# cheshmi/parsy_bench

Measured on AMD Instinct MI355X. Metric: Cholesky factorizations/sec (+ SpTRSV solves/sec), SuiteSparse SPD set, higher is better.
Workload: dtype f64; 1 GPU; flan-class stand-in (BASELINE.json configs[2] when flan: Flan_1565): grid (116, 116, 116) 27-point stencil, geometric nested dissection; n=1560896, nnz_A_lower=21491316, nsuper=81191, nnz_L=2044454227, xsize=2421483055, etree_levels=17, launches_per_factorization=356, parallelism=1 GPU

## Files before the change

parsy_bench_amd/csrc/schedule.cpp:

```cpp
#include "schedule.hpp"

#include <array>
#include <cstdio>
#include <map>
#include <algorithm>
#include <queue>
#include <climits>
#include <cmath>
#include <cstdlib>
#include <cstdint>
#include <functional>
#include <stdexcept>
#include <string>

namespace parsy {

static inline int ceil_div(int a, int b) { return (a + b - 1) / b; }

static int env_int(const char* name, int dflt) {
    const char* v = std::getenv(name);
    if (!v || !*v) return dflt;
    return std::atoi(v);
}

static int find_subtrees(const std::vector<int>& parent, const std::vector<uint8_t>& eligible,
                         const std::vector<double>& cost, double cap, std::vector<int32_t>& subtree,
                         const std::vector<std::pair<int32_t, int32_t>>* slots = nullptr, int64_t slot_cap = 0) {
    const int ns = (int)parent.size();
    subtree.assign(ns, -1);
    std::vector<uint8_t> whole(eligible);
    std::vector<double> sub(cost);
    std::vector<int64_t> cols(slots ? ns : 0);
    for (int s = 0; s < ns && slots; ++s) cols[s] = (*slots)[s].first;
    for (int s = 0; s < ns; ++s) {
        const int p = parent[s];
        if (p < 0) continue;
        if (p <= s) return 0;
        if (!whole[s]) whole[p] = 0;
        sub[p] += sub[s];
        if (slots) cols[p] += cols[s];
    }
    int count = 0;
    for (int s = ns - 1; s >= 0; --s) {
        const int p = parent[s];
        if (p >= 0 && subtree[p] >= 0) subtree[s] = subtree[p];
        else if (whole[s] && sub[s] <= cap && (!slots || cols[s] + (*slots)[s].second <= slot_cap)) subtree[s] = count++;
    }
    return count;
}

namespace {

struct BuildKnobs {
    bool big_mink_set;
    int big_mink;
    bool piece_width_set;
    int piece_width;
    int push_group;
    bool split_chunks_set;
    int split_chunks;
    int split_target;
    int split_max;
    bool subtrees_set;
    int subtrees_per_cu;
    int chol_subtrees_per_cu;
    int super_r, super_c;
    int64_t super_min_tasks;
    double super_max_fill;
    int super_hi;
    int dense_mode;
    double dense_min_share;
    double dense_all_share;
    int dense_fill_min;
    bool dense_strips;
    bool big_recut;
};

BuildKnobs read_build_knobs() {
    auto percent = [](const char* name, double dflt) { return env_int(name, (int)(dflt * 100 + 0.5)); };
    BuildKnobs K{};
    K.big_mink_set = std::getenv("PARSY_BIG_MINK") != nullptr;
    K.big_mink = std::max(1, env_int("PARSY_BIG_MINK", kBigMinK));
    K.piece_width_set = std::getenv("PARSY_PIECE_WIDTH") != nullptr;
    K.piece_width = env_int("PARSY_PIECE_WIDTH", kPieceWidth);
    K.push_group = std::max(1, env_int("PARSY_PUSH_GROUP", kPushGroup));
    K.split_chunks_set = std::getenv("PARSY_SPLIT_CHUNKS") != nullptr;
    K.split_chunks = env_int("PARSY_SPLIT_CHUNKS", kSplitChunks);
    K.split_target = std::max(1, env_int("PARSY_SPLIT_TARGET", kSplitTarget));
    K.split_max = std::max(1, env_int("PARSY_SPLIT_MAX", kSplitMaxParts));
    K.subtrees_set = std::getenv("PARSY_SUBTREES") != nullptr;
    K.subtrees_per_cu = env_int("PARSY_SUBTREES", kSubtreesPerCu);
    K.chol_subtrees_per_cu = std::max(1, env_int("PARSY_CHOL_SUBTREES", kCholSubtreesPerCu));
    if (const char* e = std::getenv("PARSY_BIG_SUPER")) {
        int a = 0, b = 0;
        const int got = std::sscanf(e, "%dx%d", &a, &b);
        if (got >= 1 && a >= 1 && a <= 64) {
            K.super_r = a;
            K.super_c = (got == 2 && b >= 1 && b <= 64) ? b : a;
        }
    }
    K.super_min_tasks = env_int("PARSY_BIG_SUPER_MIN", kBigSuperMinTasks);
    K.super_max_fill = percent("PARSY_BIG_SUPER_FILL", kBigSuperMaxFill) / 100.0;
    K.super_hi = std::max(1, std::min(8, env_int("PARSY_BIG_SUPER_HI", 2)));
    K.dense_mode = env_int("PARSY_BIG_DENSE", 1);
    K.dense_min_share = percent("PARSY_DENSE_MIN_SHARE", kDenseMinShare) / 100.0;
    K.dense_all_share = percent("PARSY_DENSE_ALL_SHARE", kDenseAllShare) / 100.0;
    K.dense_fill_min = percent("PARSY_DENSE_FILL", kDenseMinFill) * kBigTile * kBigTile / 100;
    K.dense_strips = env_int("PARSY_DENSE_STRIPS", 1) != 0;
    K.big_recut = env_int("PARSY_BIG_RECUT", 1) != 0;
    return K;
}

struct BigKeyed { int64_t launch_tile, window; WaveEntry e; int16_t sr, sc; };

struct BuildState {
    BuildKnobs knobs;
    int compute_units = 0;
    std::vector<int> tree;
    std::vector<int64_t> uptr, urel;
    std::vector<int> usn, ulb, uub;
    std::vector<int8_t> launch_super;
    std::vector<int64_t> level_tiles;
    std::vector<int64_t> big_tile0;
    std::vector<int32_t> upd_domain;
    std::vector<BigKeyed> bigk;
};

struct RowRun { int32_t win, first, len; };

inline int rel_at(const Schedule& S, const SnDesc& T, const UpdDesc& U, int k) {
    return U.rel < 0 ? k : S.relpos[(size_t)U.rel + k] - T.rbias;
}

void row_runs(const Schedule& S, const SnDesc& T, const UpdDesc& U, int window, std::vector<RowRun>& out) {
    out.clear();
    for (int k = 0; k < U.m;) {
        const int win = rel_at(S, T, U, k) / window;
        int k1 = k + 1;
        while (k1 < U.m && rel_at(S, T, U, k1) / window == win) ++k1;
        out.push_back(RowRun{win, k, k1 - k});
        k = k1;
    }
}

inline bool is_big(const Schedule& S, const UpdDesc& U, int target_piece) {
    const int real = S.csn_real[target_piece];
    return U.rel < 0 || U.K >= S.big_min_k || S.piece0[real + 1] - S.piece0[real] > 1;
}

inline int64_t big_launch_of(int lev_s, int lev_t) { return (int64_t)lev_s * 2 + (lev_s == lev_t - 1 ? 0 : 1); }

double block_pairs(int ia, int mi, int ja, int nj) {
    double pairs = 0;
    for (int jj = ja; jj < ja + nj; ++jj) pairs += std::max(0, ia + mi - std::max(ia, jj));
    return pairs;
}

void describe_supernodes(const PatternRef& P, const size_t* lC, const int* A2p, Schedule& S) {
    const int n = P.n, ns = P.nsuper;
    S.n = n;
    S.nsuper = ns;
    S.solve_only = (A2p == nullptr);
    S.nnzA = A2p ? A2p[n] : 0;
    S.rows.assign(P.s, P.s + P.i_ptr[n]);
    S.ssize = (int64_t)P.i_ptr[n];
    S.xsize = (int64_t)lC[n];
    S.sn.resize(ns);
    for (int t = 0; t < ns; ++t) {
        SnDesc& d = S.sn[t];
        d.c0 = P.super[t];
        d.w = P.super[t + 1] - P.super[t];
        d.r = (int)(P.i_ptr[P.super[t + 1]] - P.i_ptr[P.super[t]]);
        d.ld = d.r;
        d.rbias = 0;
        d.px = (int64_t)lC[d.c0];
        d.pi = (int64_t)P.i_ptr[d.c0];
        d.a0 = A2p ? A2p[d.c0] : 0;
        d.a1 = A2p ? A2p[P.super[t + 1]] : 0;
        d.upd0 = 0;
        d.nupd = 0;
        d.dslot = -1;
        d.tflag0 = -1;
        if (d.w <= 0 || d.r < d.w) throw std::runtime_error("schedule: malformed supernode");
        if ((int64_t)d.w * d.r > 0x7fffffffLL)
            throw std::runtime_error("schedule: a single panel exceeds 2^31 entries");
        for (int col = d.c0; col < d.c0 + d.w; ++col)
            if (lC[col + 1] - lC[col] != (size_t)d.r || P.i_ptr[col] != P.i_ptr[d.c0])
                throw std::runtime_error("schedule: lC / Li_ptr are not a column-major panel layout");
        S.max_width = std::max(S.max_width, d.w);
        S.max_rows = std::max(S.max_rows, d.r);
        S.nnzL += (int64_t)d.w * d.r - (int64_t)d.w * (d.w - 1) / 2;
        for (int k = 0; k < d.w; ++k) S.flops_stored += (double)(d.r - k) * (double)(d.r - k);
        for (int k = 0; k < d.w; ++k)
            if (S.rows[d.pi + k] != d.c0 + k)
                throw std::runtime_error("schedule: supernode rows do not start with its own columns");
        if (d.w > kTile) {
            d.dslot = (int32_t)S.n_dslots;
            S.n_dslots += ceil_div(d.w, kTile);
        }
    }
}

void list_updates(const PatternRef& P, const size_t* lC, const int* A2p, const int* A2i, Schedule& S, BuildState& B) {
    const int n = P.n, ns = P.nsuper;
    B.uptr.assign(ns + 1, 0);
    if (!S.solve_only) build_update_lists(P, B.uptr, B.usn, B.ulb, B.uub);
    B.urel.assign(B.usn.size(), 0);
// ... 300 lines not shown
                    rg[part * 8 + 2 * q + 1] = e;
                }
            }
            tsplit[tp / 2] = (int64_t)S.split_desc.size();
            S.split_desc.push_back(sd);
        }
    }
}

void build_wave_streams(Schedule& S, BuildState& B) {
    const int nc = (int)S.csn.size();
    S.sn_wp0.assign(nc, -1);
    S.sn_tw0.assign(nc, -1);
    B.level_tiles.assign((size_t)std::max(S.cnlevels, 1), 0);
    if (S.solve_only) return;
    for (int t = 0; t < nc; ++t)
        if (!is_small(S.csn[t])) {
            const int nbc = ceil_div(S.csn[t].w, kTile), nbr = ceil_div(S.csn[t].r, kTile);
            B.level_tiles[(size_t)S.level_of[t]] += (int64_t)nbc * nbr - (int64_t)nbc * (nbc - 1) / 2;
        }
    std::vector<RowRun> runs;
    std::vector<int64_t> cursor;
    for (int t = 0; t < nc; ++t) {
        SnDesc& T = S.csn[t];
        if (is_small(T)) {
            S.n_small++;
            continue;
        }
        S.n_big++;
        const int nbc = ceil_div(T.w, kTile), nbr = ceil_div(T.r, kTile);
        if (S.n_tflags + (int64_t)nbc * nbr > 0x7fffffffLL) throw std::runtime_error("schedule: too many tiles");
        T.tflag0 = (int32_t)S.n_tflags;
        S.n_tflags += (int64_t)nbc * nbr;
        for (int jb = 1; jb < nbc; ++jb) {
            const double K = (double)jb * kTile, wb = std::min(kTile, T.w - jb * kTile);
            S.inner_flops += K * wb * (wb + 1) + 2.0 * K * (double)(T.r - jb * kTile - wb) * wb;
        }
        piece_wave_streams(S, t, runs, cursor);
        piece_tile_weights(S, B, t);
    }
}

template <class Fn>
void tile_cut_blocks(const Schedule& S, const SnDesc& T, const UpdDesc& U, int sr, int sc, std::vector<RowRun>& runs,
                     std::vector<RowRun>& cruns, Fn&& fn) {
    row_runs(S, T, U, kBigTile * sr, runs);
    if (sc == sr) cruns = runs;
    else row_runs(S, T, U, kBigTile * sc, cruns);
    for (const RowRun& gc : cruns) {
        if (gc.first >= U.n1) break;
        const int njt = std::min(gc.len, U.n1 - gc.first);
        for (const RowRun& gr : runs) {
            if ((int64_t)(gr.win + 1) * sr * kBigTile - 1 < (int64_t)gc.win * sc * kBigTile) continue;
            for (int cb = 0; cb < njt; cb += kBigTile)
                for (int rb = 0; rb < gr.len; rb += kBigTile) {
                    const int mi = std::min(kBigTile, gr.len - rb), nj = std::min(kBigTile, njt - cb);
                    const int ia = gr.first + rb, ja = gc.first + cb;
                    if (ia + mi - 1 < ja) continue;
                    fn(gr.win, gc.win, ia, mi, ja, nj);
                }
        }
    }
}

template <class Fn>
void recut_blocks(const UpdDesc& U, bool strips, Fn&& fn) {
    strips = strips && U.K >= kDenseChunk;
    for (int ja = 0; ja < U.n1; ja += kBigTile)
        for (int ia = ja; ia < U.m; ia += kBigTile) {
            const int mi = std::min(kBigTile, U.m - ia), nj = std::min(kBigTile, U.n1 - ja);
            const bool row_strip = strips && mi <= kStripMax && nj == kBigTile && ia >= ja + kBigTile;
            const bool col_strip = strips && !row_strip && nj <= kStripMax && mi == kBigTile && ja >= kBigTile;
            fn(ia / kBigTile - row_strip, ja / kBigTile - col_strip, ia, mi, ja, nj, row_strip || col_strip);
        }
}

int64_t issued_ns(const BuildKnobs& K, int mi, int nj, int k, bool rides) {
    if (rides) return (int64_t)ceil_div(k, kDenseChunk) * kIssueStripNs;
    const bool dense = K.dense_mode != 0 && k >= kDenseChunk && (K.dense_mode == 4 || mi * nj >= K.dense_fill_min);
    if (dense) return (int64_t)ceil_div(k, kDenseChunk) * kIssueDenseNs;
    return (int64_t)ceil_div(k, 16) * (kIssueRaggedNs + (int64_t)kIssueFragmentNs * ceil_div(mi, 16) * ceil_div(nj, 16));
}

void find_conflict_domains(Schedule& S, BuildState& B) {
    const BuildKnobs& K = B.knobs;
    const int nc = (int)S.csn.size();
    B.upd_domain.assign(S.upd.size(), 0);
    if (S.solve_only || !K.big_recut) return;
    std::vector<std::pair<int64_t, int64_t>> big;
    std::vector<int64_t> owner;
    std::vector<int32_t> root;
    std::vector<std::pair<int32_t, int32_t>> members;
    std::vector<RowRun> runs, cruns;
    auto find = [&](int32_t x) {
        while (root[(size_t)x] != x) x = root[(size_t)x] = root[(size_t)root[(size_t)x]];
        return x;
    };
    for (int t = 0; t < nc; ++t) {
        const SnDesc& T = S.csn[t];
        if (is_small(T)) continue;
        big.clear();
        for (int64_t u = T.upd0; u < T.upd0 + T.nupd; ++u)
            if (is_big(S, S.upd[u], t)) big.push_back({big_launch_of(S.level_of[S.upd_src[u]], S.level_of[t]), u});
        std::stable_sort(big.begin(), big.end(), [](const auto& a, const auto& b) { return a.first < b.first; });
        owner.assign((size_t)T.w, -1);
        for (size_t i = 0; i < big.size();) {
            size_t j = i;
            while (j < big.size() && big[j].first == big[i].first) ++j;
            const int64_t launch = big[i].first;
            const int32_t nm = (int32_t)(j - i);
            root.resize((size_t)nm);
            for (int32_t q = 0; q < nm; ++q) {
                root[(size_t)q] = q;
                const UpdDesc& U = S.upd[big[i + q].second];
                for (int k = 0; k < U.n1; ++k) {
                    const int c = rel_at(S, T, U, k);
                    if (c < 0 || c >= T.w) throw std::runtime_error("schedule: a column row of an update lies outside its target");
                    int64_t& o = owner[(size_t)c];
                    if (o < 0 || (o >> 32) != launch) {
                        o = (launch << 32) | q;
                        continue;
                    }
                    const int32_t a = find(q), b = find((int32_t)(o & 0xffffffff));
                    if (a < b) root[(size_t)b] = a;
                    else root[(size_t)a] = b;
                }
            }
            const int sr = K.super_r ? K.super_r : B.launch_super[(size_t)launch];
            const int sc = K.super_r ? K.super_c : B.launch_super[(size_t)launch];
            members.clear();
            for (int32_t q = 0; q < nm; ++q) members.push_back({find(q), q});
            std::sort(members.begin(), members.end());
            for (size_t d0 = 0, d1; d0 < members.size(); d0 = d1) {
                const int32_t q = members[d0].first;
                for (d1 = d0; d1 < members.size() && members[d1].first == q; ++d1) {}
                const UpdDesc& U0 = S.upd[big[i + q].second];
                bool same = true;
                for (size_t d = d0 + 1; d < d1 && same; ++d) {
                    const UpdDesc& U = S.upd[big[i + members[d].second].second];
                    same = U.m == U0.m && U.n1 == U0.n1;
                    for (int k = 0; k < U.m && same; ++k) same = rel_at(S, T, U, k) == rel_at(S, T, U0, k);
                }
                if (!same) continue;
                int64_t tile_ns = 0, recut_ns = 0;
                for (size_t d = d0; d < d1; ++d) {
                    const UpdDesc& U = S.upd[big[i + members[d].second].second];
                    tile_cut_blocks(S, T, U, sr, sc, runs, cruns, [&](int, int, int, int mi, int, int nj) {
                        tile_ns += issued_ns(K, mi, nj, U.K, false);
                    });
                    recut_blocks(U, K.dense_strips && K.dense_mode != 0, [&](int, int, int, int mi, int, int nj, bool rides) {
                        recut_ns += issued_ns(K, mi, nj, U.K, rides);
                    });
                }
                if (recut_ns >= tile_ns) continue;
                const int64_t first = big[i + q].second - T.upd0;
                if (first >= 0x7fffffff) throw std::runtime_error("schedule: too many updates of one piece");
                for (size_t d = d0; d < d1; ++d) B.upd_domain[(size_t)big[i + members[d].second].second] = (int32_t)first + 1;
            }
            i = j;
        }
    }
}

void collect_big_entries(Schedule& S, BuildState& B) {
    const int nc = (int)S.csn.size();
    const int env_sr = B.knobs.super_r, env_sc = B.knobs.super_c;
    B.big_tile0.assign((size_t)nc + 1, 0);
    std::vector<RowRun> runs, cruns;
    for (int t = 0; t < nc; ++t) {
        const SnDesc& T = S.csn[t];
        B.big_tile0[t + 1] = B.big_tile0[t];
        if (S.solve_only || is_small(T)) continue;
        const int lev_t = S.level_of[t];
        const int nbr128 = ceil_div(T.r, kBigTile), nbc128 = ceil_div(T.w, kBigTile);
        B.big_tile0[t + 1] = B.big_tile0[t] + (int64_t)nbr128 * nbc128;
        for (int64_t u = T.upd0; u < T.upd0 + T.nupd; ++u) {
            const UpdDesc& U = S.upd[u];
            const double f = (double)U.K * U.n1 * (U.n1 + 1) + 2.0 * U.K * (double)(U.m - U.n1) * U.n1;
            if (!is_big(S, U, t)) {
                S.tile_update_flops += f;
                continue;
            }
            S.big_flops += f;
            const int lev_s = S.level_of[S.upd_src[u]];
            if (lev_s >= lev_t) throw std::runtime_error("schedule: an update source is not below its target");
            const int64_t launch = big_launch_of(lev_s, lev_t);
            const int sr = env_sr ? env_sr : B.launch_super[(size_t)launch], sc = env_sr ? env_sc : B.launch_super[(size_t)launch];
            auto entry = [&](int ia, int mi, int ja, int nj) {
                return WaveEntry{U.src, (int32_t)std::max<int64_t>(U.rel, 0), U.ld, U.K, ia, ja, mi | (nj << 8) | ((U.rel < 0) << 16)};
            };
            const int64_t domain = B.upd_domain[(size_t)u];
            if (domain) {
                if (U.m / kBigTile >= 0xffff) throw std::runtime_error("schedule: too many windows of one update");
                recut_blocks(U, B.knobs.dense_strips && B.knobs.dense_mode != 0, [&](int wr, int wc, int ia, int mi, int ja, int nj, bool) {
                    B.bigk.push_back(BigKeyed{(launch << 40) | B.big_tile0[t], (domain << 32) | ((int64_t)wc << 16) | wr,
                                              entry(ia, mi, ja, nj), 1, 1});
                });
                continue;
            }
            tile_cut_blocks(S, T, U, sr, sc, runs, cruns, [&](int wr, int wc, int ia, int mi, int ja, int nj) {
                const int64_t tile = B.big_tile0[t] + (int64_t)wc * sc * nbr128 + (int64_t)wr * sr;
                B.bigk.push_back(BigKeyed{(launch << 40) | tile, 0, entry(ia, mi, ja, nj), (int16_t)sr, (int16_t)sc});
            });
        }
    }
}

std::vector<uint8_t> dense_share_per_launch(const BuildState& B) {
    const BuildKnobs& K = B.knobs;
    std::vector<double> lprod(B.launch_super.size(), 0.0), ldense(B.launch_super.size(), 0.0);
    for (const BigKeyed& b : B.bigk) {
        const WaveEntry& E = b.e;
        const size_t l = (size_t)(b.launch_tile >> 40);
        const double products = (double)ceil_div(E.K, 4) * ceil_div(entry_rows(E), 16) * ceil_div(entry_cols(E), 16);
        lprod[l] += products;
        if (entry_rows(E) == kBigTile && entry_cols(E) == kBigTile && E.K >= kDenseChunk) ldense[l] += products;
    }
    std::vector<uint8_t> launch_dense(B.launch_super.size(), 0);
    for (size_t l = 0; l < launch_dense.size(); ++l) {
        if (K.dense_mode == 4) {
            launch_dense[l] = lprod[l] > 0 ? 2 : 0;
            continue;
        }
        if (K.dense_mode == 0 || ldense[l] <= 0) continue;
        if (K.dense_mode >= 2 || ldense[l] >= K.dense_min_share * lprod[l]) launch_dense[l] = 1;
        if (launch_dense[l] && lprod[l] - ldense[l] <= K.dense_all_share * lprod[l] && K.dense_mode != 3) launch_dense[l] = 2;
    }
    return launch_dense;
}

void build_big_tasks(Schedule& S, BuildState& B) {
    std::vector<BigKeyed>& bigk = B.bigk;
    if (bigk.empty()) return;
    const int nc = (int)S.csn.size();
    std::stable_sort(bigk.begin(), bigk.end(),
                     [](const BigKeyed& a, const BigKeyed& b) {
                         return a.launch_tile != b.launch_tile ? a.launch_tile < b.launch_tile : a.window < b.window;
                     });
    const std::vector<uint8_t> launch_dense = dense_share_per_launch(B);
    const int fill_min = B.knobs.dense_fill_min;
    auto is_dense = [fill_min](const WaveEntry& E, int mode) {
        if (mode == 2) return E.K >= kDenseChunk;
        return mode == 1 && E.K >= kDenseChunk && entry_rows(E) * entry_cols(E) >= fill_min;
    };
    S.big_entries.resize(bigk.size());
    std::map<std::pair<int64_t, int64_t>, size_t> strip_of;
    std::vector<uint8_t> absorbed;
    int t = 0;
    for (size_t i = 0; i < bigk.size();) {
        size_t j = i;
        while (j < bigk.size() && bigk[j].launch_tile == bigk[i].launch_tile && bigk[j].window == bigk[i].window) ++j;
        const int64_t launch = bigk[i].launch_tile >> 40, tile = bigk[i].launch_tile & ((1LL << 40) - 1);
        size_t at = i;
        int64_t weight = 0, dweight = 0, dchunks = 0;
        const int lmode = launch_dense[(size_t)launch];
        const bool strips_ride = bigk[i].window != 0 && lmode == 2 && B.knobs.dense_strips;
        auto dense_here = [&](const WaveEntry& E) {
            if (!is_dense(E, lmode)) return false;
            const int mi = entry_rows(E), nj = entry_cols(E);
            return !(strips_ride && ((mi <= kStripMax && nj == kBigTile) || (nj <= kStripMax && mi == kBigTile)));
        };
        if (lmode)
            for (size_t q = i; q < j; ++q) {
                const WaveEntry& E = bigk[q].e;
                if (!dense_here(E)) continue;
                S.big_entries[at++] = E;
                dchunks += ceil_div(E.K, kDenseChunk);
                dweight += ceil_div(E.K, 16) + 2;
                S.dense_flops += 2.0 * E.K * block_pairs(E.ia, entry_rows(E), E.ja, entry_cols(E));
            }
        const size_t mid = at;
        int32_t nstrips = 0;
        absorbed.assign(j - i, 0);
        if (lmode && B.knobs.dense_strips && mid > i) {
            strip_of.clear();
            for (size_t d = i; d < mid; ++d) {
                const WaveEntry& E = S.big_entries[d];
                if ((E.mn & 0xffff) == (kBigTile | (kBigTile << 8))) strip_of[{E.src, ((int64_t)E.ia << 32) | (uint32_t)E.ja}] = d;
            }
            for (size_t q = i; q < j && !strip_of.empty(); ++q) {
                const WaveEntry& R = bigk[q].e;
                if (dense_here(R)) continue;
                const int mi = entry_rows(R), nj = entry_cols(R);
                const bool row_strip = mi <= kStripMax && nj == kBigTile, col_strip = nj <= kStripMax && mi == kBigTile;
                if (!row_strip && !col_strip) continue;
                const auto it = strip_of.find({R.src, ((int64_t)(R.ia - (row_strip ? kBigTile : 0)) << 32) |
                                                      (uint32_t)(R.ja - (col_strip ? kBigTile : 0))});
                if (it == strip_of.end()) continue;
                WaveEntry& E = S.big_entries[it->second];
                if (E.K != R.K || big_ident(E) != big_ident(R) || E.rel != R.rel || E.ld != R.ld) continue;
                if ((row_strip ? big_strip_rows(E) : big_strip_cols(E)) != 0) continue;
                if (big_strip_rows(E) == 0 && big_strip_cols(E) == 0) ++nstrips;
                E.mn |= row_strip ? mi << 17 : nj << 22;
                absorbed[q - i] = 1;
                S.dense_flops += 2.0 * R.K * block_pairs(R.ia, mi, R.ja, nj);
                dweight += ceil_div(R.K, 64);
            }
        }
        for (size_t q = i; q < j; ++q)
            if (!dense_here(bigk[q].e) && !absorbed[q - i]) {
                S.big_entries[at++] = bigk[q].e;
                weight += ceil_div(bigk[q].e.K, 16) + 4;
            }
        const size_t jend = at;
        S.n_dense_entries += (int64_t)(mid - i);
        S.n_strip_entries += nstrips;
        while (t + 1 < nc && B.big_tile0[t + 1] <= tile) ++t;
        if (tile < B.big_tile0[t]) {
            t = 0;
            while (B.big_tile0[t + 1] <= tile) ++t;
        }
        const int nbr128 = ceil_div(S.csn[t].r, kBigTile);
        const int64_t local = tile - B.big_tile0[t];
        const int64_t window = bigk[i].window;
        const int32_t row0 = window ? (int32_t)(window & 0xffff) * kBigTile : (int32_t)(local % nbr128) * kBigTile;
        const int32_t col0 = window ? (int32_t)((window >> 16) & 0xffff) * kBigTile : (int32_t)(local / nbr128) * kBigTile;
        S.big_all.push_back(Schedule::BigTask{t, row0, col0,
                                              (int32_t)std::min<int64_t>(weight, INT32_MAX), (int64_t)i, (int64_t)jend,
                                              (int32_t)(launch >> 1), (int32_t)((launch & 1) == 0), bigk[i].sr, bigk[i].sc,
                                              (int64_t)mid, (int32_t)std::min<int64_t>(dweight, INT32_MAX),
                                              (int32_t)std::min<int64_t>(dchunks, INT32_MAX), nstrips, (int32_t)(window >> 32)});
        i = j;
    }
}

}

void build_schedule(const PatternRef& P, const size_t* lC, const int* A2p, const int* A2i,
                    const uint8_t* active, Schedule& S, int compute_units) {
    S = Schedule();
    BuildState B;
    B.knobs = read_build_knobs();
    B.compute_units = compute_units;
    if (compute_units > 0) S.walker_batch = std::max(4, std::min(kWalkerBatch, compute_units / 2));
    describe_supernodes(P, lC, A2p, S);
    list_updates(P, lC, A2p, A2i, S, B);
    choose_sizes(S, B.knobs);
    cut_pieces(P, S, B);
    describe_updates(S, B);
// ... 1350 lines not shown
            if (l.rows_only != 0 && !(l.rows_only == 1 && k == kLaunchChain)) fail(who + "rows_only is set");
            if (l.ticket != 0 && !(k == kLaunchChain || chain_form)) fail(who + "has a ticket counter but takes no tickets");
            if (l.ticket < 0 || (l.ticket > 0 && l.ticket >= ntickets)) fail(who + "ticket counter " + std::to_string(l.ticket) + " does not exist");
            if ((l.lds_bytes != 0 || l.stage != 0) && k != kLaunchSmall) fail(who + "lds_bytes / stage are set");
            if (l.lds_bytes < 0 || l.stage < 0) fail(who + "negative lds_bytes / stage");
            if (l.width != 0 && k != kLaunchSolveSmall) fail(who + "width is set");
            if (l.width_class < 0 || l.width_class > 2 || (l.width_class != 0 && k != kLaunchBackBlock))
                fail(who + "width_class = " + std::to_string(l.width_class));
            if ((l.task_first != 0 || l.task_count != 0) && !chain_form) fail(who + "has a task range but is no chain-form launch");
        }
    };
    check_list(S.chol, "chol", [](int k) { return is_chol_launch(k); }, S.n_chain_launches);
    check_list(S.solve, "solve", [](int k) { return k == kLaunchSolveSmall || k == kLaunchSolvePanel || k == kLaunchSolveFixup; },
               S.n_solve_chain_launches);
    check_list(S.bsolve, "bsolve", [](int k) { return k == kLaunchBackBelow || k == kLaunchBackBlock; }, S.n_solve_chain_launches);
}

int64_t check_schedule(const Schedule& S, std::string& what) {
    int64_t bad = 0;
    auto fail = [&](const std::string& msg) {
        if (bad++ == 0) what = msg;
    };
    check_launch_records(S, fail);
    check_solve_launches(S, fail);
    check_solve_one(S, fail);
    check_sub_tiers(S, fail);
    if (S.solve_only) return bad;
    const int nc = (int)S.csn.size();
    for (int t = 0; t < S.nsuper; ++t) {
        int cols = 0;
        for (int p = S.piece0[t]; p < S.piece0[t + 1]; ++p) {
            const SnDesc& C = S.csn[p];
            if (C.c0 != S.sn[t].c0 + cols || C.rbias != cols || C.r != S.sn[t].r - cols || C.ld != S.sn[t].r)
                fail("piece " + std::to_string(p) + " is not a window of its supernode's panel");
            if (p > S.piece0[t] && S.level_of[p] != S.level_of[p - 1] + 1) fail("pieces of a supernode are not on consecutive levels");
            cols += C.w;
        }
        if (cols != S.sn[t].w) fail("pieces of supernode " + std::to_string(t) + " do not add up to its width");
    }
    std::vector<double> covered(S.upd.size(), 0.0);
    auto entry_flops = [](const WaveEntry& E, bool same_window) {
        const double K = E.K, mi = E.mn & 255, nj = (E.mn >> 8) & 255;
        return same_window ? K * nj * (nj + 1) + 2.0 * K * (mi - nj) * nj : 2.0 * K * mi * nj;
    };
    auto block_flops = [](const WaveEntry& E) {
        const int mi = E.mn & 255, nj = (E.mn >> 8) & 255;
        auto pairs_of = [](int ia, int m, int ja, int n) {
            double pairs = 0;
            for (int j = ja; j < ja + n; ++j) pairs += std::max(0, ia + m - std::max(ia, j));
            return pairs;
        };
        return 2.0 * E.K * (pairs_of(E.ia, mi, E.ja, nj) + pairs_of(E.ia + mi, big_strip_rows(E), E.ja, nj) +
                            pairs_of(E.ia, mi, E.ja + nj, big_strip_cols(E)));
    };
    for (int t = 0; t < nc; ++t) {
        const SnDesc& T = S.csn[t];
        for (int64_t u = T.upd0; u < T.upd0 + T.nupd; ++u)
            if (S.level_of[S.upd_src[u]] >= S.level_of[t]) fail("update " + std::to_string(u) + " comes from a level that is not below its target");
        if (is_small(T) || T.nupd == 0) continue;
        auto find_upd = [&](const WaveEntry& E) -> int64_t {
            for (int64_t u = T.upd0; u < T.upd0 + T.nupd; ++u)
                if (S.upd[u].src == E.src && S.upd[u].K == E.K) return u;
            return -1;
        };
        if (S.sn_wp0[t] >= 0) {
            const int nbc = ceil_div(T.w, kTile), nbr = ceil_div(T.r, kTile);
            const int64_t* wp = &S.wave_ptr[S.sn_wp0[t]];
            for (size_t key = 0; key < (size_t)nbc * nbr * 8; ++key)
                for (int64_t e = wp[key]; e < wp[key + 1]; ++e) {
                    const WaveEntry& E = S.wave_entries[(size_t)e];
                    const int64_t u = find_upd(E);
                    const int mi = E.mn & 255, nj = (E.mn >> 8) & 255;
                    if (u < 0 || mi < 1 || mi > kSub || nj < 1 || nj > kSub || E.ia + mi > S.upd[u].m || E.ja + nj > S.upd[u].n1) {
                        fail("wave entry " + std::to_string(e) + " of piece " + std::to_string(t) + " has a bad window");
                        continue;
                    }
                    covered[(size_t)u] += entry_flops(E, E.ia == E.ja);
                }
        }
    }
    std::vector<int32_t> col_domain;
    std::map<int32_t, int64_t> domain_upd;
    std::vector<std::array<int32_t, 3>> domain_wins;
    const Schedule::BigTask* group = nullptr;
    auto close_group = [&]() {
        std::sort(domain_wins.begin(), domain_wins.end());
        if (std::adjacent_find(domain_wins.begin(), domain_wins.end()) != domain_wins.end())
            fail("two BIG tasks of piece " + std::to_string(group->sn) + " own the same window of a conflict domain");
        domain_wins.clear();
        domain_upd.clear();
    };
    for (const Schedule::BigTask& b : S.big_all) {
        const SnDesc& T = S.csn[b.sn];
        if (b.src_level >= S.level_of[b.sn] || (b.next != 0) != (b.src_level == S.level_of[b.sn] - 1))
            fail("BIG task of piece " + std::to_string(b.sn) + " is filed under the wrong source level");
        if (!group || group->sn != b.sn || group->src_level != b.src_level || group->next != b.next) {
            if (group) close_group();
            group = &b;
            col_domain.assign((size_t)T.w, -1);
        }
        const int win_r = kBigTile * b.sr, win_c = kBigTile * b.sc;
        if (b.domain < 0 || b.sr < 1 || b.sc < 1 || b.row0 % win_r || b.col0 % win_c || b.row0 + win_r <= b.col0 ||
            (b.domain ? b.sr != 1 || b.sc != 1 : b.row0 >= T.r || b.col0 >= T.w))
            fail("BIG task of piece " + std::to_string(b.sn) + " has a bad tile origin");
        if (b.domain) domain_wins.push_back({b.domain, b.row0, b.col0});
        for (int64_t e = b.e0; e < b.e1; ++e) {
            const WaveEntry& E = S.big_entries[(size_t)e];
            int64_t u = -1;
            for (int64_t q = T.upd0; q < T.upd0 + T.nupd; ++q)
                if (S.upd[q].src == E.src && S.upd[q].K == E.K) u = q;
            const int mi = E.mn & 255, nj = (E.mn >> 8) & 255;
            const bool ident = big_ident(E);
            const int ms = big_strip_rows(E), ns = big_strip_cols(E);
            if ((ms || ns) && (e >= b.em || mi != kBigTile || nj != kBigTile || ms > kStripMax || ns > kStripMax))
                fail("BIG entry " + std::to_string(e) + " carries a strip but is not a full dense block");
            if (u < 0 || mi < 1 || mi > kBigTile || nj < 1 || nj > kBigTile || E.ia + mi + ms > S.upd[u].m || E.ja + nj + ns > S.upd[u].n1 ||
                ident != (S.upd[u].rel < 0) || S.level_of[S.upd_src[u]] != b.src_level) {
                fail("BIG entry " + std::to_string(e) + " of piece " + std::to_string(b.sn) + " has a bad window or source");
                continue;
            }
            auto rel_at = [&](int k) { return ident ? k : S.relpos[(size_t)S.upd[u].rel + k] - T.rbias; };
            for (int k = E.ja; k < E.ja + nj + ns; ++k) {
                int32_t& d = col_domain[(size_t)rel_at(k)];
                if (d >= 0 && d != b.domain)
                    fail("column " + std::to_string(rel_at(k)) + " of piece " + std::to_string(b.sn) + " belongs to two conflict domains of a launch");
                d = b.domain;
            }
            if (!b.domain) {
                if (rel_at(E.ia) / win_r != b.row0 / win_r || rel_at(E.ia + mi + ms - 1) / win_r != b.row0 / win_r ||
                    rel_at(E.ja) / win_c != b.col0 / win_c || rel_at(E.ja + nj + ns - 1) / win_c != b.col0 / win_c)
                    fail("BIG entry " + std::to_string(e) + " names rows outside its task's tile");
            } else {
                const UpdDesc& U = S.upd[u];
                auto inside = [](int first, int count, int win0, int len) {
                    const int end = first + count, wend = win0 + kBigTile;
                    return first >= win0 && (end <= wend || (end <= len && len - wend <= kStripMax));
                };
                if (!inside(E.ia, mi + ms, b.row0, U.m) || !inside(E.ja, nj + ns, b.col0, U.n1))
                    fail("BIG entry " + std::to_string(e) + " names rows outside its task's window");
                const UpdDesc& U0 = S.upd[(size_t)domain_upd.emplace(b.domain, u).first->second];
                bool same = U.m == U0.m && U.n1 == U0.n1 && (U.rel < 0) == (U0.rel < 0);
                if (&U != &U0 && !ident) {
                    for (int k = E.ia; k < E.ia + mi + ms && same; ++k) same = S.relpos[(size_t)U.rel + k] == S.relpos[(size_t)U0.rel + k];
                    for (int k = E.ja; k < E.ja + nj + ns && same; ++k) same = S.relpos[(size_t)U.rel + k] == S.relpos[(size_t)U0.rel + k];
                }
                if (!same) fail("BIG entry " + std::to_string(e) + ": the members of its conflict domain do not have the same rows");
            }
            covered[(size_t)u] += block_flops(E);
        }
    }
    if (group) close_group();
    {
        std::vector<int64_t> starts;
        std::vector<int64_t> dense_pos(S.big_all.size(), -1), ragged_pos(S.big_all.size(), -1);
        int64_t li = 0;
        for (const Launch& l : S.chol) {
            ++li;
            if (l.kind != kLaunchBig && l.kind != kLaunchDense) continue;
            const bool dense = l.kind == kLaunchDense;
            const bool side = l.side != 0;
            auto find_task = [&](int64_t e) -> const Schedule::BigTask* {
                auto it = std::upper_bound(S.big_all.begin(), S.big_all.end(), e,
                                           [](int64_t v, const Schedule::BigTask& b) { return v < b.e0; });
                if (it == S.big_all.begin()) return nullptr;
                --it;
                return e < it->e1 ? &*it : nullptr;
            };
            auto right_launch = [&](const Schedule::BigTask& b) {
                return side != (b.next != 0) && (side ? l.wait_level : l.level - 1) == b.src_level;
            };
            for (int q = l.first; q < l.first + l.count; ++q) {
                const TileDesc& td = S.big_tasks[(size_t)q];
                if (td.wp >= td.sp) {
                    if (td.wp != td.sp) fail("BIG launch task " + std::to_string(q) + " has a negative entry range");
                    continue;
                }
                const Schedule::BigTask* it = find_task(td.wp);
                const bool ok = it && (dense ? (it->e0 == td.wp && it->em == td.sp && (td.part & ~kDenseStripTask) == it->dchunks &&
                                                ((td.part & kDenseStripTask) != 0) == (it->strips > 0))
                                             : (it->em == td.wp && it->e1 == td.sp));
                if (!ok || it->sn != td.sn || it->row0 != td.row0 || it->col0 != td.col0) {
                    fail("BIG launch task " + std::to_string(q) + " is not a task of the plan");
                    continue;
                }
                if (!right_launch(*it)) fail("BIG launch task " + std::to_string(q) + " runs in the launch of another source level");
                (dense ? dense_pos : ragged_pos)[(size_t)(it - S.big_all.data())] = li;
                starts.push_back(td.wp);
            }
        }
        std::sort(starts.begin(), starts.end());
        if (std::adjacent_find(starts.begin(), starts.end()) != starts.end()) fail("a BIG task is launched twice");
        int64_t want = 0;
        for (size_t k = 0; k < S.big_all.size(); ++k) {
            const Schedule::BigTask& b = S.big_all[k];
            if (b.em < b.e0 || b.em > b.e1) fail("BIG task " + std::to_string(k) + " has a bad dense / ragged split");
            int64_t dch = 0;
            int32_t nst = 0;
            for (int64_t e = b.e0; e < b.em; ++e) {
                const WaveEntry& E = S.big_entries[(size_t)e];
                nst += big_strip_rows(E) || big_strip_cols(E);
                if (E.K < kDenseChunk) fail("BIG entry " + std::to_string(e) + " is filed as dense but is narrower than a chunk");
                dch += ceil_div(E.K, kDenseChunk);
            }
            if (dch != b.dchunks) fail("BIG task " + std::to_string(k) + " has a wrong dense chunk count");
            if (nst != b.strips) fail("BIG task " + std::to_string(k) + " has a wrong count of entries with strips");
            if (!S.active_piece[b.sn]) continue;
            want += (b.em > b.e0) + (b.e1 > b.em);
            if (b.em > b.e0 && b.e1 > b.em && !(dense_pos[k] > 0 && ragged_pos[k] > dense_pos[k]))
                fail("BIG task " + std::to_string(k) + ": the ragged part is not launched after the dense part");
        }
        if ((int64_t)starts.size() != want)
            fail("BIG launches hold " + std::to_string(starts.size()) + " task parts, the active targets have " + std::to_string(want));
    }
    for (int t = 0; t < nc; ++t) {
// ... 62 lines not shown
```

parsy_bench_amd/csrc/schedule.hpp:

```cpp
#pragma once
#include <cstddef>
#include <cstdint>
#include <string>
#include <vector>

#include "inspector.hpp"

namespace parsy {

constexpr int kTile = 64;
constexpr int kSub = 32;
constexpr int kSmallMaxEntries = 6144;
constexpr int kSmallMaxWidth = 64;
constexpr int kBelowRows = 512;
constexpr int kBelowMaxGroups = 512;
constexpr int kBackGroup = 2;
constexpr int kTinyWidth = 16;
constexpr int kTinyWidth2 = 32;
constexpr int kPanelRows = 128;
constexpr int kSolveRows = 256;
constexpr int kSolveRowsMrhs = 128;

struct SnDesc {
    int64_t px;
    int64_t pi;
    int64_t upd0;
    int32_t c0, w, r;
    int32_t nupd;
    int32_t a0, a1;
    int32_t dslot;
    int32_t tflag0;
    int32_t ld;
    int32_t rbias;
};

struct UpdDesc {
    int64_t src;
    int64_t rel;
    int32_t ld;
    int32_t K;
    int32_t m;
    int32_t n1;
};

struct WaveEntry {
    int64_t src;
    int32_t rel;
    int32_t ld, K;
    int32_t ia, ja;
    int32_t mn;
};
constexpr int kStripMax = 16;
constexpr int kIssueDenseNs = 2090, kIssueStripNs = 260, kIssueRaggedNs = 1000, kIssueFragmentNs = 60;
inline int entry_rows(const WaveEntry& E) { return E.mn & 255; }
inline int entry_cols(const WaveEntry& E) { return (E.mn >> 8) & 255; }
inline bool big_ident(const WaveEntry& E) { return (E.mn >> 16) & 1; }
inline int big_strip_rows(const WaveEntry& E) { return (E.mn >> 17) & 31; }
inline int big_strip_cols(const WaveEntry& E) { return (E.mn >> 22) & 31; }
constexpr int kDenseStripTask = 1 << 30;

struct TileDesc {
    int32_t sn;
    int32_t row0, col0;
    int32_t part;
    int64_t wp;
    int64_t sp;
};

struct PanelDesc {
    int32_t sn;
    int32_t jb;
    int32_t row0;
    int32_t pad;
};

struct SubMember {
    int64_t px;
    int32_t c0, w, r;
    int32_t slot0;
    int32_t so;
    int32_t ld;
};
struct SubTree {
    int32_t m0, m1;
    int32_t ncols;
    int32_t nout;
    int32_t out0;
    int32_t pad[3];
};
struct SubTier {
    int32_t tree0, ntrees;
    int32_t max_slots;
    int32_t top_level;
};
constexpr int kSubMaxSlots = 320;
constexpr int kSubTierMaxWidth = 64;
constexpr int kSubTierMinTrees = 512;
constexpr int kSubTierMaxSlots = 448;
constexpr int kSubTierMaxDensity = 700;

enum LaunchKind : int32_t {
    kLaunchSmall = 0, kLaunchTiles = 1, kLaunchChain = 2, kLaunchBig = 3,
    kLaunchBackBelow = 4,
    kLaunchSolveSmall = 5, kLaunchSolvePanel = 6, kLaunchSolveFixup = 7, kLaunchBackBlock = 8,
    kLaunchDense = 9,
};
inline bool is_chol_launch(int kind) { return (kind >= 0 && kind <= kLaunchBig) || kind == kLaunchDense; }

enum LaunchForm : int32_t {
    kFormEach = 0,
    kFormChain = 1,
    kFormSubtrees = 2,
};

struct Launch {
    int32_t kind;
    int32_t first = 0, count = 0;
    int32_t level = 0;
    int32_t side = 0;
    int32_t wait_level = -1;
    int32_t form = kFormEach;
    int32_t rows_only = 0;
    int32_t ticket = 0;
    int32_t lds_bytes = 0;
    int32_t stage = 0;
    int32_t width = 0;
    int32_t width_class = 0;
    int32_t task_first = 0, task_count = 0;
};
constexpr int kLaunchFields = 15;
static_assert(sizeof(Launch) == kLaunchFields * sizeof(int32_t), "Launch: fields and kLaunchFields disagree");

constexpr int kSplitChunks = 192;
constexpr int kSplitTarget = 128;
constexpr int kSplitMaxParts = 4;
constexpr int kSplitFewTiles = 128;
// ... 151 lines not shown
```

Measured before the change: 3.036 factorizations/s.

## Recut non-identical BIG update conflict domains into swept row intervals

Adds an interval-based recut mode for conflict domains whose member updates have different row patterns. Row boundaries come from a sweep that caps each update at one block per interval. The cut is used only when its estimated issue cost beats the tiled cut and it does not lengthen the longest task beyond the launch's share across issue slots. The aim is to pack ragged updates into fuller blocks and cut fragment overhead, at the cost of more schedule-build work, a new domain encoding, and checker logic for interval overlap.

```diff
diff --git a/parsy_bench_amd/csrc/schedule.cpp b/parsy_bench_amd/csrc/schedule.cpp
--- a/parsy_bench_amd/csrc/schedule.cpp
+++ b/parsy_bench_amd/csrc/schedule.cpp
@@ -5,6 +5,7 @@
 #include <map>
 #include <algorithm>
 #include <queue>
+#include <set>
 #include <climits>
 #include <cmath>
 #include <cstdlib>
@@ -73,7 +74,8 @@
     double dense_all_share;
     int dense_fill_min;
     bool dense_strips;
-    bool big_recut;
+    bool big_recut_set;
+    int big_recut;
 };
 
 BuildKnobs read_build_knobs() {
@@ -107,7 +109,8 @@
     K.dense_all_share = percent("PARSY_DENSE_ALL_SHARE", kDenseAllShare) / 100.0;
     K.dense_fill_min = percent("PARSY_DENSE_FILL", kDenseMinFill) * kBigTile * kBigTile / 100;
     K.dense_strips = env_int("PARSY_DENSE_STRIPS", 1) != 0;
-    K.big_recut = env_int("PARSY_BIG_RECUT", 1) != 0;
+    K.big_recut_set = std::getenv("PARSY_BIG_RECUT") != nullptr;
+    K.big_recut = std::max(0, std::min(3, env_int("PARSY_BIG_RECUT", 2)));
     return K;
 }
 
@@ -123,6 +126,8 @@
     std::vector<int64_t> level_tiles;
     std::vector<int64_t> big_tile0;
     std::vector<int32_t> upd_domain;
+    std::vector<int64_t> upd_bounds;
+    std::vector<int32_t> bounds;
     std::vector<BigKeyed> bigk;
 };
 
@@ -589,16 +594,95 @@
     return (int64_t)ceil_div(k, 16) * (kIssueRaggedNs + (int64_t)kIssueFragmentNs * ceil_div(mi, 16) * ceil_div(nj, 16));
 }
 
+void interval_bounds(const Schedule& S, const SnDesc& T, const std::vector<const UpdDesc*>& members,
+                     std::vector<std::pair<int32_t, int32_t>>& rows, std::vector<int32_t>& count, std::vector<int32_t>& bounds) {
+    rows.clear();
+    for (size_t q = 0; q < members.size(); ++q)
+        for (int k = 0; k < members[q]->m; ++k) rows.push_back({rel_at(S, T, *members[q], k), (int32_t)q});
+    std::sort(rows.begin(), rows.end());
+    count.assign(members.size(), 0);
+    bounds.assign(1, 0);
+    for (size_t a = 0, b; a < rows.size(); a = b) {
+        const int32_t pos = rows[a].first;
+        for (b = a; b < rows.size() && rows[b].first == pos; ++b) {}
+        int32_t start = 0;
+        if (pos >= T.w && bounds.back() < T.w) start = T.w;
+        for (size_t c = a; c < b && !start; ++c)
+            if (count[(size_t)rows[c].second] == kBigTile) start = pos;
+        if (start) {
+            bounds.push_back(start);
+            std::fill(count.begin(), count.end(), 0);
+        }
+        for (size_t c = a; c < b; ++c) ++count[(size_t)rows[c].second];
+    }
+}
+
+template <class Fn>
+void interval_blocks(const Schedule& S, const SnDesc& T, const UpdDesc& U, const int32_t* bounds, int nb, std::vector<RowRun>& runs,
+                     Fn&& fn) {
+    runs.clear();
+    int w = 0;
+    for (int k = 0; k < U.m;) {
+        const int pos = rel_at(S, T, U, k);
+        while (w + 1 < nb && bounds[w + 1] <= pos) ++w;
+        int k1 = k + 1;
+        while (k1 < U.m && (w + 1 >= nb || rel_at(S, T, U, k1) < bounds[w + 1])) ++k1;
+        if (k1 - k > kBigTile) throw std::runtime_error("schedule: an interval holds more than a block of one update's rows");
+        runs.push_back(RowRun{w, k, k1 - k});
+        k = k1;
+    }
+    for (const RowRun& gc : runs) {
+        if (gc.first >= U.n1) break;
+        const int nj = std::min(gc.len, U.n1 - gc.first);
+        for (const RowRun& gr : runs) {
+            if (gr.win < gc.win || gr.first + gr.len - 1 < gc.first) continue;
+            fn(gr.win, gc.win, gr.first, gr.len, gc.first, nj);
+        }
+    }
+}
+
 void find_conflict_domains(Schedule& S, BuildState& B) {
     const BuildKnobs& K = B.knobs;
     const int nc = (int)S.csn.size();
     B.upd_domain.assign(S.upd.size(), 0);
-    if (S.solve_only || !K.big_recut) return;
+    B.upd_bounds.assign(S.upd.size(), -1);
+    B.bounds.clear();
+    const int recut = K.big_recut_set || (S.update_flops >= kPieceAutoFlops && !K.super_r) ? K.big_recut : 1;
+    if (S.solve_only || !recut) return;
+    std::vector<RowRun> runs, cruns;
+    auto super_of = [&](int64_t launch) {
+        return std::pair<int, int>{K.super_r ? K.super_r : B.launch_super[(size_t)launch], K.super_r ? K.super_c : B.launch_super[(size_t)launch]};
+    };
+    std::vector<int64_t> launch_tile_ns(B.launch_super.size(), 0);
+    if (recut == 2)
+        for (int t = 0; t < nc; ++t) {
+            const SnDesc& T = S.csn[t];
+            if (is_small(T)) continue;
+            for (int64_t u = T.upd0; u < T.upd0 + T.nupd; ++u) {
+                const UpdDesc& U = S.upd[u];
+                if (!is_big(S, U, t)) continue;
+                const int64_t launch = big_launch_of(S.level_of[S.upd_src[u]], S.level_of[t]);
+                const auto [sr, sc] = super_of(launch);
+                int64_t ns = 0;
+                tile_cut_blocks(S, T, U, sr, sc, runs, cruns, [&](int, int, int, int mi, int, int nj) { ns += issued_ns(K, mi, nj, U.K, false); });
+                launch_tile_ns[(size_t)launch] += ns;
+            }
+        }
+    std::vector<const UpdDesc*> member_upd;
+    std::vector<std::pair<int32_t, int32_t>> sweep_rows;
+    std::vector<int32_t> sweep_count, ivals;
+    std::map<std::pair<int, int>, int64_t> tile_task, ival_task;
+    std::set<std::array<int, 4>> full_blocks;
+    const bool strips = K.dense_mode != 0;
+    auto longest = [](const std::map<std::pair<int, int>, int64_t>& m) {
+        int64_t v = 0;
+        for (const auto& kv : m) v = std::max(v, kv.second);
+        return v;
+    };
     std::vector<std::pair<int64_t, int64_t>> big;
     std::vector<int64_t> owner;
     std::vector<int32_t> root;
     std::vector<std::pair<int32_t, int32_t>> members;
-    std::vector<RowRun> runs, cruns;
     auto find = [&](int32_t x) {
         while (root[(size_t)x] != x) x = root[(size_t)x] = root[(size_t)root[(size_t)x]];
         return x;
@@ -633,8 +717,7 @@
                     else root[(size_t)a] = b;
                 }
             }
-            const int sr = K.super_r ? K.super_r : B.launch_super[(size_t)launch];
-            const int sc = K.super_r ? K.super_c : B.launch_super[(size_t)launch];
+            const auto [sr, sc] = super_of(launch);
             members.clear();
             for (int32_t q = 0; q < nm; ++q) members.push_back({find(q), q});
             std::sort(members.begin(), members.end());
@@ -648,7 +731,48 @@
                     same = U.m == U0.m && U.n1 == U0.n1;
                     for (int k = 0; k < U.m && same; ++k) same = rel_at(S, T, U, k) == rel_at(S, T, U0, k);
                 }
-                if (!same) continue;
+                const int64_t first = big[i + q].second - T.upd0;
+                if (first >= kIntervalDomain - 1) throw std::runtime_error("schedule: too many updates of one piece");
+                if (!same) {
+                    if (recut < 2) continue;
+                    member_upd.clear();
+                    for (size_t d = d0; d < d1; ++d) member_upd.push_back(&S.upd[big[i + members[d].second].second]);
+                    interval_bounds(S, T, member_upd, sweep_rows, sweep_count, ivals);
+                    if (ivals.size() >= 0xffff) throw std::runtime_error("schedule: too many intervals of one conflict domain");
+                    tile_task.clear();
+                    ival_task.clear();
+                    int64_t tile_ns = 0, ival_ns = 0;
+                    for (const UpdDesc* U : member_upd) {
+                        full_blocks.clear();
+                        tile_cut_blocks(S, T, *U, sr, sc, runs, cruns, [&](int wr, int wc, int ia, int mi, int ja, int nj) {
+                            const bool row_strip = mi <= kStripMax && nj == kBigTile, col_strip = nj <= kStripMax && mi == kBigTile;
+                            if (mi == kBigTile && nj == kBigTile) full_blocks.insert({wr, wc, ia, ja});
+                            const bool rides = strips && U->K >= kDenseChunk && (row_strip || col_strip) &&
+                                               full_blocks.count({wr, wc, ia - (row_strip ? kBigTile : 0), ja - (col_strip ? kBigTile : 0)}) != 0;
+                            const int64_t ns = issued_ns(K, mi, nj, U->K, rides);
+                            tile_ns += ns;
+                            tile_task[{wr, wc}] += ns;
+                        });
+                        interval_blocks(S, T, *U, ivals.data(), (int)ivals.size(), runs, [&](int wr, int wc, int, int mi, int, int nj) {
+                            const int64_t ns = issued_ns(K, mi, nj, U->K, false);
+                            ival_ns += ns;
+                            ival_task[{wr, wc}] += ns;
+                        });
+                    }
+                    if (ival_ns >= tile_ns) continue;
+                    if (recut == 2 &&
+                        longest(ival_task) > std::max(longest(tile_task), launch_tile_ns[(size_t)launch] / kIssueSlots))
+                        continue;
+                    const int64_t at = (int64_t)B.bounds.size();
+                    B.bounds.push_back((int32_t)ivals.size());
+                    B.bounds.insert(B.bounds.end(), ivals.begin(), ivals.end());
+                    for (size_t d = d0; d < d1; ++d) {
+                        const size_t u = (size_t)big[i + members[d].second].second;
+                        B.upd_domain[u] = kIntervalDomain + (int32_t)first + 1;
+                        B.upd_bounds[u] = at;
+                    }
+                    continue;
+                }
                 int64_t tile_ns = 0, recut_ns = 0;
                 for (size_t d = d0; d < d1; ++d) {
                     const UpdDesc& U = S.upd[big[i + members[d].second].second];
@@ -660,8 +784,6 @@
                     });
                 }
                 if (recut_ns >= tile_ns) continue;
-                const int64_t first = big[i + q].second - T.upd0;
-                if (first >= 0x7fffffff) throw std::runtime_error("schedule: too many updates of one piece");
                 for (size_t d = d0; d < d1; ++d) B.upd_domain[(size_t)big[i + members[d].second].second] = (int32_t)first + 1;
             }
             i = j;
@@ -697,6 +819,14 @@
                 return WaveEntry{U.src, (int32_t)std::max<int64_t>(U.rel, 0), U.ld, U.K, ia, ja, mi | (nj << 8) | ((U.rel < 0) << 16)};
             };
             const int64_t domain = B.upd_domain[(size_t)u];
+            if (domain >= kIntervalDomain) {
+                const int32_t* iv = &B.bounds[(size_t)B.upd_bounds[(size_t)u]];
+                interval_blocks(S, T, U, iv + 1, iv[0], runs, [&](int wr, int wc, int ia, int mi, int ja, int nj) {
+                    B.bigk.push_back(BigKeyed{(launch << 40) | B.big_tile0[t], (domain << 32) | ((int64_t)wc << 16) | wr,
+                                              entry(ia, mi, ja, nj), 1, 1});
+                });
+                continue;
+            }
             if (domain) {
                 if (U.m / kBigTile >= 0xffff) throw std::runtime_error("schedule: too many windows of one update");
                 recut_blocks(U, B.knobs.dense_strips && B.knobs.dense_mode != 0, [&](int wr, int wc, int ia, int mi, int ja, int nj, bool) {
@@ -761,7 +891,7 @@
         size_t at = i;
         int64_t weight = 0, dweight = 0, dchunks = 0;
         const int lmode = launch_dense[(size_t)launch];
-        const bool strips_ride = bigk[i].window != 0 && lmode == 2 && B.knobs.dense_strips;
+        const bool strips_ride = bigk[i].window != 0 && (bigk[i].window >> 32) < kIntervalDomain && lmode == 2 && B.knobs.dense_strips;
         auto dense_here = [&](const WaveEntry& E) {
             if (!is_dense(E, lmode)) return false;
             const int mi = entry_rows(E), nj = entry_cols(E);
@@ -2278,8 +2408,17 @@
     std::vector<int32_t> col_domain;
     std::map<int32_t, int64_t> domain_upd;
     std::vector<std::array<int32_t, 3>> domain_wins;
+    std::map<std::pair<int32_t, int32_t>, std::pair<int32_t, int32_t>> ival_span;
     const Schedule::BigTask* group = nullptr;
     auto close_group = [&]() {
+        int32_t dom = 0, top = -1;
+        for (const auto& kv : ival_span) {
+            if (kv.first.first != dom) dom = kv.first.first, top = -1;
+            if (kv.second.first <= top)
+                fail("intervals " + std::to_string(kv.first.second) + " and below of a conflict domain of piece " + std::to_string(group->sn) + " overlap");
+            top = std::max(top, kv.second.second);
+        }
+        ival_span.clear();
         std::sort(domain_wins.begin(), domain_wins.end());
         if (std::adjacent_find(domain_wins.begin(), domain_wins.end()) != domain_wins.end())
             fail("two BIG tasks of piece " + std::to_string(group->sn) + " own the same window of a conflict domain");
@@ -2326,6 +2465,14 @@
                 if (rel_at(E.ia) / win_r != b.row0 / win_r || rel_at(E.ia + mi + ms - 1) / win_r != b.row0 / win_r ||
                     rel_at(E.ja) / win_c != b.col0 / win_c || rel_at(E.ja + nj + ns - 1) / win_c != b.col0 / win_c)
                     fail("BIG entry " + std::to_string(e) + " names rows outside its task's tile");
+            } else if (b.domain >= kIntervalDomain) {
+                auto name = [&](int32_t index, int k0, int k1) {
+                    auto& span = ival_span.emplace(std::make_pair(b.domain, index), std::make_pair(INT32_MAX, -1)).first->second;
+                    span.first = std::min(span.first, (int32_t)rel_at(k0));
+                    span.second = std::max(span.second, (int32_t)rel_at(k1 - 1));
+                };
+                name(b.row0 / kBigTile, E.ia, E.ia + mi + ms);
+                name(b.col0 / kBigTile, E.ja, E.ja + nj + ns);
             } else {
                 const UpdDesc& U = S.upd[u];
                 auto inside = [](int first, int count, int win0, int len) {
diff --git a/parsy_bench_amd/csrc/schedule.hpp b/parsy_bench_amd/csrc/schedule.hpp
--- a/parsy_bench_amd/csrc/schedule.hpp
+++ b/parsy_bench_amd/csrc/schedule.hpp
@@ -52,6 +52,8 @@
 };
 constexpr int kStripMax = 16;
 constexpr int kIssueDenseNs = 2090, kIssueStripNs = 260, kIssueRaggedNs = 1000, kIssueFragmentNs = 60;
+constexpr int kIssueSlots = 512;
+constexpr int32_t kIntervalDomain = 1 << 30;
 inline int entry_rows(const WaveEntry& E) { return E.mn & 255; }
 inline int entry_cols(const WaveEntry& E) { return (E.mn >> 8) & 255; }
 inline bool big_ident(const WaveEntry& E) { return (E.mn >> 16) & 1; }
```

Measured after the change: 3.149 factorizations/s (median of 6 runs). +3.7%, better.
